# esteinig/sketchy

Measured on AMD Instinct MI355X. Metric: reads/sec streamed (s=10000,k=16,40k-genome ref), higher is better.
Workload: dtype u64

## Files before the change

sketchy_amd/csrc/skx_capi.hip:

```cpp
#include <dlfcn.h>
#include <hip/hip_runtime.h>
#include <rccl/rccl.h>

#include <unistd.h>

#include <algorithm>
#include <atomic>
#include <chrono>
#include <cmath>
#include <condition_variable>
#include <cstdarg>
#include <cstdio>
#include <cstdlib>
#include <cstring>
#include <mutex>
#include <string>
#include <thread>
#include <unordered_map>
#include <vector>

#include "sketchy_hip.h"
#include "skx_common.hpp"
#include "skx_kernels.hpp"

// ... 899 lines not shown
    bool back_pending[2] = {false, false};
    hipEvent_t ev_pslot[3] = {nullptr, nullptr, nullptr};
    bool pslot_pending[3] = {false, false, false};
    int pslot = 0;
    hipEvent_t ev_pairq[2] = {nullptr, nullptr};
    bool pairq_pending[2] = {false, false};
    bool packed = false;
    u32 top_k = 0, max_reads = 0, sk_stride = 0;
    u64 max_bases = 0;
    u32 pcap = 0;
    u32 qcap = 0;
    u64* d_qd = nullptr;
    u32 *d_qrow = nullptr, *d_sslot = nullptr, *d_qinfo = nullptr, *d_qloc = nullptr, *d_cls_bsum = nullptr;
    u32* d_nd_hs = nullptr;
    u32* h_lcount = nullptr;
    u32 lcount_seq = 0, lcount_seen = 0, lcount_floor = 0;
    u32* h_nq_sink = nullptr;
    u32* h_nd = nullptr;
    u32 *d_rowcnt = nullptr;
    u32 *d_gain = nullptr;
    u32 *d_gain_s = nullptr;
    u32 *d_candslot = nullptr;
    u32 *d_candmask = nullptr;
    uint2 *d_lrow = nullptr;
    u32 *d_nlrow = nullptr, *d_gain_l = nullptr, *d_cbase = nullptr, *d_cwl = nullptr, *d_ncwl = nullptr;
    u64 *d_cw = nullptr;
    u64 *d_inb = nullptr, *d_hit = nullptr;
    skx::LongRows long_rows() const { return skx::LongRows{d_lrow, d_nlrow, qcap + 128, d_inb, ref->n_lw}; }
    bool use_pat = false;
    u32 *d_hist = nullptr, *d_nprow = nullptr;
    u64* d_pcw = nullptr;
    u32 npat_pad = 0;
    skx::PatRows pat_rows() const { return skx::PatRows{d_hist, npat_pad, d_gain_l, d_nprow}; }
    skx::RareIndex rare_index() const {
        skx::RareIndex ri = ref->rare_index();
        if (!use_pat) { ri.prec = nullptr; ri.n_pat = 0; }
        if (!static_dense) { ri.qs = nullptr; ri.n_sd = 0; }
        return ri;
    }
    u32 *d_cbad = nullptr, *d_nqc = nullptr;
    u32 *d_spc_g0 = nullptr, *d_spc_grp = nullptr;
    u32 n_pad_c = 0, n_grp_c = 0, cand_seq = 0;
    struct PassSet {
        u64 *tab = nullptr;
        u32 *cand = nullptr;
        u64 *tabc = nullptr;
        u32 *ncand = nullptr;
        u32 *mode = nullptr, *any_full = nullptr, *nqc_total = nullptr;
        u64 *mc = nullptr;
        u64 *mqc = nullptr;
        u64 *rowany_c = nullptr;
        u32 *grp_any_c = nullptr;
        u32 *smap = nullptr;
        u32 *pair_qc = nullptr;
        u32 *nd = nullptr;
        u32 *h_pub = nullptr;
    } ps[2];
    struct PassChains {
        bool pending = false, ranked = false, has_cand = false, update_table = false, forced_full = false, legacy = false;
        SubPass subs[kGroupMax];
        int n_sub = 0, b = 0, slot = 0;
        u32 P = 0, nq_rows = 0, seq = 0;
        u64 nq_est = 0;
    } pcq[2];
    int pc_head = 0, pc_n = 0;
    bool hint_all_overflow = false;
    u32 hint_seq = 0;
    u32 passes_since_fresh = 0;
    bool fresh_table = true;
    u32 legacy_run = 0;
    u64 batches_compact = 0, batches_full = 0;
    bool have_split_hint = false;
    double nd_frac = 1.0;
    u32 qcap_max = 0;
    bool qcap_auto = false;
    u64 qrows_grown = 0;
    u32 coalesce = 1;
    u32 rpass = 0;
    u64 reads_total = 0;
    uint8_t* d_bases = nullptr;
    u64* d_offsets = nullptr;
    u64* d_sk = nullptr;
    u32 *d_len = nullptr, *d_cnt = nullptr, *d_poff = nullptr;
    bool side_ready[kSides] = {};
    u64* sd_sk[kSides] = {};
    u64 pool_cap[kSides] = {};
    u32 pool_fixed = 0;
    u64* sd_rows[kSides] = {};
    u32 cur_stride = 0;
    u32 cur_pool_cap = 0, cur_pool_fixed = 0;
// ... 112 lines not shown
    std::vector<hipEvent_t> ev_pool;
    double ms[SKX_N_STAGES] = {0, 0, 0, 0, 0};
    u64 launches[SKX_N_STAGES] = {0, 0, 0, 0, 0};
};

static void free_side(skx_stream* st, int i);
static void free_lane(skx_stream* st, int i);
static void stream_free(skx_stream* st) {
    if (!st) return;
    (void)hipSetDevice(st->device);
    if (st->hs0) (void)hipStreamSynchronize(st->hs0);
    if (st->hs1) (void)hipStreamSynchronize(st->hs1);
    if (st->hs) (void)hipStreamSynchronize(st->hs);
    if (st->hs2) (void)hipStreamSynchronize(st->hs2);
    for (int i = 1; i < skx_stream::kRankLanes; ++i)
        if (st->lane[i].s) (void)hipStreamSynchronize(st->lane[i].s);
    for (int i = 0; i < kSides; ++i) (void)hipFree(st->sd_rows[i]);
    void* ptrs[] = {st->d_bases, st->d_offsets, st->d_pair_h[0], st->d_pair_h[1],
                    st->d_q[0], st->d_q[1], st->d_pair_r[0], st->d_pair_r[1], st->d_pair_q[0], st->d_pair_q[1],
                    st->d_poff_pass[0], st->d_poff_pass[1], st->d_poff_pass[2], st->d_pair_r[2], st->d_nq[0], st->d_nq[1], st->d_win[0], st->d_win[1], st->d_m, st->d_mint, st->d_mq[0], st->d_mq[1],
                    st->d_topk_idx, st->d_topk_sum, st->d_cons, st->d_ev.n_events, st->d_ev.ev_read, st->d_ev.ev_idx, st->d_ev.ev_sum, st->d_ev.ev_codes, st->d_tab_tmp, st->d_rank_idx, st->d_rank_sum, st->d_bsum, st->d_grp_any[0],
                    st->d_grp_any[1], st->d_hbuf, st->d_wb[0], st->d_wb[1], st->d_rowany[0], st->d_rowany[1], st->d_mqext,
                    st->d_qd, st->d_qrow, st->d_sslot, st->d_qinfo, st->d_qloc, st->d_cls_bsum, st->d_nd_hs,
                    st->d_rowcnt, st->d_gain, st->d_gain_s, st->d_candslot, st->d_candmask, st->d_lrow, st->d_nlrow, st->d_gain_l, st->d_cbase, st->d_cwl, st->d_ncwl, st->d_cw, st->d_cbad, st->d_nqc, st->d_spc_g0, st->d_spc_grp, st->d_inb, st->d_hit, st->d_hist, st->d_nprow, st->d_pcw, st->d_ms[0], st->d_ms[1], st->d_mdirty_s};
    for (auto& q : st->ps) {
        for (void* x : {(void*)q.tab, (void*)q.cand, (void*)q.tabc, (void*)q.ncand, (void*)q.mode, (void*)q.any_full, (void*)q.nqc_total, (void*)q.mc, (void*)q.mqc,
                        (void*)q.rowany_c, (void*)q.grp_any_c, (void*)q.smap, (void*)q.pair_qc, (void*)q.nd}) (void)hipFree(x);
        if (q.h_pub) (void)hipHostFree(q.h_pub);
    }
    for (auto& t : st->d_tab) (void)hipFree(t);
    for (int i = 0; i < skx_stream::kRankLanes; ++i) free_lane(st, i);
    for (int i = 1; i < skx_stream::kRankLanes; ++i)
        if (st->own_lane_stream && st->lane[i].s) (void)hipStreamDestroy(st->lane[i].s);
    for (void* p : ptrs) (void)hipFree(p);
    if (st->h_poff) (void)hipHostFree(st->h_poff);
    if (st->h_offsets) (void)hipHostFree(st->h_offsets);
    if (st->h_nq) (void)hipHostFree(st->h_nq);
    if (st->h_nd) (void)hipHostFree(st->h_nd);
    if (st->h_nq_sink) (void)hipHostFree(st->h_nq_sink);
    if (st->h_lcount) (void)hipHostFree(st->h_lcount);
    if (st->h_chk_base) (void)hipHostFree(st->h_chk_base);
    for (int i = 0; i < kSides; ++i) {
        free_side(st, i);
        if (st->ev_main[i]) (void)hipEventDestroy(st->ev_main[i]);
    }
    if (!st->shared_queues && st->hs1 && st->hs1 != st->hs0) (void)hipStreamDestroy(st->hs1);
    (void)hipFree(st->d_ht[0]); (void)hipFree(st->d_ht[1]); (void)hipFree(st->d_dict_ctr[0]); (void)hipFree(st->d_dict_ctr[1]);
// ... 392 lines not shown
    memset(st->h_nd, 0, 4 * 4);
    SCHK(hipHostMalloc((void**)&st->h_nq_sink, 4 * 4, hipHostMallocCoherent));
    SCHK(hipHostMalloc((void**)&st->h_lcount, 4 * 4, hipHostMallocCoherent));
    memset(st->h_lcount, 0, 4 * 4);
    SCHK(hipMalloc(&st->d_nd_hs, 64));
    SCHK(hipMemset(st->d_nd_hs, 0, 64));
    if (ref->d_kt_key) {
        SCHK(hipMalloc(&st->d_qd, (size_t)st->pcap * 8));
        SCHK(hipMalloc(&st->d_qrow, (size_t)st->pcap * 4));
        SCHK(hipMalloc(&st->d_sslot, (size_t)st->pcap * 8));
        SCHK(hipMalloc(&st->d_qinfo, (size_t)st->pcap * 4));
        SCHK(hipMalloc(&st->d_qloc, (size_t)st->pcap * 4));
        SCHK(hipMalloc(&st->d_cls_bsum, ((size_t)st->pcap / 1024 + 2) * 4));
    }
    {
        const u32 nb = skx::kPassBatchesMax, cap = skx::kCandCap, rows_c = skx::kCandRows;
        st->n_pad_c = n_sp * cap;
        st->n_grp_c = st->n_pad_c / (skx::kRankWords * 64);
        SCHK(hipMalloc(&st->d_rowcnt, (size_t)nb * ((size_t)st->qcap + 128) * 4));
        SCHK(hipMalloc(&st->d_gain, (size_t)nb * n_pad * 4));
        if (ref->d_kt_key) SCHK(hipMalloc(&st->d_gain_s, (size_t)nb * n_pad * 4 * skx::gain_sparse_stride()));
        SCHK(hipMalloc(&st->d_candslot, (size_t)nb * n_pad * 4));
        SCHK(hipMalloc(&st->d_candmask, (size_t)n_pad * 4));
        if (ref->d_mlong) {
            SCHK(hipMalloc(&st->d_lrow, (size_t)nb * ((size_t)st->qcap + 128) * 8));
            SCHK(hipMalloc(&st->d_nlrow, skx::pass_counter_bytes()));
            SCHK(hipMalloc(&st->d_gain_l, (size_t)nb * n_pad * 4));
            SCHK(hipMalloc(&st->d_cw, (size_t)nb * (n_pad / 64) * 8));
            SCHK(hipMalloc(&st->d_cbase, (size_t)nb * (n_pad / 64) * 4));
            SCHK(hipMalloc(&st->d_cwl, (size_t)nb * st->n_pad_c * 4));
            SCHK(hipMalloc(&st->d_ncwl, 64));
            if (ref->d_mlongT) {
                SCHK(hipMalloc(&st->d_inb, (size_t)nb * ref->n_lw * 8));
                SCHK(hipMalloc(&st->d_hit, (size_t)nb * ref->n_lw * 8));
            }
            if (ref->d_prec && ref->n_pat && st->n_grp_c * skx::kRankWords <= skx::pat_words_max()) {
                st->use_pat = true;
                st->npat_pad = (ref->n_pat + 63u) & ~63u;
                SCHK(hipMalloc(&st->d_hist, (size_t)nb * st->npat_pad * 4));
                SCHK(hipMalloc(&st->d_nprow, skx::pass_counter_bytes()));
                SCHK(hipMalloc(&st->d_pcw, (size_t)nb * ref->n_pat * st->n_grp_c * skx::kRankWords * 8));
            }
        }
        SCHK(hipMalloc(&st->d_cbad, 64));
        SCHK(hipMalloc(&st->d_nqc, skx::pass_counter_bytes()));
        std::vector<u32> g0c(n_sp), grpc(st->n_grp_c);
// ... 274 lines not shown
        st->hint_pairs[b] = P;
    }
    if (P == 0) HIPCHK(hipMemsetAsync(d_nd, 0, 16, hs));
    HIPCHK(hipGetLastError());
    if (!inserted) {
        HIPCHK(hipEventRecord(st->ev_skread[st->side], hs));
        st->sk_reader_pending[st->side] = true;
    }
    HIPCHK(hipEventRecord(st->ev_dict[b], hs));

    if (!sdm && ((!st->have_hint && !nq_known && P > 0) || (split_dict && !st->have_split_hint && P > 0))) {
        HIPCHK(hipStreamSynchronize(hs));
        take_hint(b, P);
        st->have_split_hint = true;
        if (!nq_known) nq_est = std::max<u64>(1, hint_nq(b));
    }
    const u64 nd_est = sdm ? std::max<u32>(1u, ref->n_sd) : split_dict ? std::max<u64>(1, (u64)((double)nq_est * st->nd_frac * 1.1) + 64) : nq_est;

    const u32 n_grp_all = n_pad / (skx::kRankWords * 64);
    u32* d_mdirty = d_grp_any + n_grp_all;
    SKX_MARK("pass: dictionary queued", 0);
    HIPCHK(hipMemsetAsync(d_mdirty, 0, 4, hs));
    SKX_MARK("pass: memset mdirty", 0);
    auto wait_back = [&]() -> int {
        if (st->back_pending[b]) { HIPCHK(hipStreamWaitEvent(hs, st->ev_back[b], 0)); st->back_pending[b] = false; }
        HIPCHK(hipMemcpyAsync(ps.nd, d_nd, 16, hipMemcpyDeviceToDevice, hs));
        HIPCHK(hipMemsetAsync(d_grp_any, 0, (size_t)n_grp_all * 4, hs));
        if (P > 0) {
            skx::launch_pair_q(hs, st->d_pair_h[b], P, d_q, d_nq, d_pair_q, split_dict ? st->d_qrow : nullptr, st->d_bbase, st->d_btot, ref->max_ref);
            HIPCHK(hipGetLastError());
        }
        HIPCHK(hipEventRecord(st->ev_pairq[b], hs));
        st->pairq_pending[b] = true;
        return SKX_OK;
    };
    bool ranked = false, all_forced = false, all_ranked = true;
    for (int i = 0; i < n_sub; ++i) {
        const bool r = st->top_k && subs[i].d_topk_idx && subs[i].d_topk_sum;
        ranked = ranked || r; all_ranked = all_ranked && r && !subs[i].d_shared && !subs[i].d_counts;
    }
    const u32* only_if = nullptr;
    u32 seq = 0;
    static const int legacy_env = skx::knob("SKX_TABLE_LEGACY") ? atoi(skx::knob("SKX_TABLE_LEGACY")) : 1 << 30;
    static const int cand_env0 = skx::knob("SKX_CAND") ? atoi(skx::knob("SKX_CAND")) : 1;
    const bool fresh_overflow = st->fresh_table && ref->max_species > skx::kCandCap && st->top_k <= 1;
    const bool second_blind = st->passes_since_fresh == 1 && !((int)(st->lcount_seen - st->lcount_floor) > 0);
    const bool legacy = update_table && all_ranked && cand_env0 && legacy_env > 0 &&
                        (fresh_overflow || (st->hint_all_overflow && !second_blind && (int)st->legacy_run < legacy_env));
    st->legacy_run = legacy ? st->legacy_run + 1 : 0;
    if (update_table) { st->passes_since_fresh = st->fresh_table ? 1 : st->passes_since_fresh + 1; st->fresh_table = false; }
    const bool long_rows = split_dict && ref->d_mlong != nullptr;
    static const int tail_env = skx::knob("SKX_TAIL_SCALE") ? atoi(skx::knob("SKX_TAIL_SCALE")) : 8;
    const u32 walk_scale = st->tail_pass ? (u32)std::max(1, tail_env) : 1u;
    skx::PassBatches pbt;
    pbt.n = (u32)n_sub;
    for (int i = 0; i < n_sub; ++i) pbt.p_off[i] = subs[i].p_off;
    pbt.p_off[n_sub] = P;
    auto rare_gains = [&](hipStream_t on) -> int {
        const skx::RareIndex ri = st->rare_index();
        const skx::LongRows lrows = st->long_rows();
        const skx::PatRows prows = st->pat_rows();
        skx::launch_gain_sparse(on, d_nd, q_bound, st->d_rowcnt, qstride, (u32)n_sub, n_pad, st->d_gain_s, st->d_sslot, ri, long_rows ? &lrows : nullptr, walk_scale,
                                (long_rows && st->use_pat) ? &prows : nullptr);
        if (long_rows) skx::launch_gain_long(on, lrows, ri, d_nd, st->d_rowcnt, qstride, (u32)n_sub, n_pad, st->d_gain_l, walk_scale);
        if (long_rows && st->use_pat)
            skx::launch_gain_dense(on, ri.pm, nullptr, n_pad, ri.d_npat, ri.n_pat, st->d_hist, st->npat_pad, (u32)n_sub, st->d_gain_l);
        HIPCHK(hipGetLastError());
        return SKX_OK;
    };
    auto row_counts = [&]() -> int {
        HIPCHK(hipMemset2DAsync(st->d_rowcnt, (size_t)qstride * 4, 0, (size_t)nq_rows * 4, (size_t)n_sub, hs));
        skx::launch_pass_hist(hs, d_pair_q, pbt, st->d_rowcnt, qstride);
// ... 62 lines not shown
        const u64* m_int = split ? st->d_mint : nullptr;
        HIPCHK(hipMemsetAsync(st->d_gain, 0, (size_t)n_sub * n_pad * 4, hs));
        if (P > 0) {
            SKXCHK(row_counts());
            skx::launch_gain_dense(hs, d_m, m_int, n_pad, d_nd, sdm ? ref->n_sd : q_bound, st->d_rowcnt, qstride, (u32)n_sub, st->d_gain,
                                   (sdm && ref->n_species > 1) ? ref->d_segw : nullptr, ref->d_grp_sp);
            if (split_dict) SKXCHK(rare_gains(hs));
        }
        skx::launch_pass_tables(hs, st->d_cum, st->d_gain, (split_dict && P > 0) ? st->d_gain_s : nullptr,
                                (long_rows && P > 0) ? st->d_gain_l : nullptr, (u32)n_sub, n_pad, ps.tab);
        st->d_cum = ps.tab + (size_t)n_sub * n_pad;
        static const int cand_env = skx::knob("SKX_CAND") ? atoi(skx::knob("SKX_CAND")) : 1;
        static const int hint_env = skx::knob("SKX_CAND_HINT") ? atoi(skx::knob("SKX_CAND_HINT")) : 1;
        (void)hint_env;
        all_forced = !cand_env;
        u32 force_full = all_forced ? 0xFFu : 0u;
        for (int i = 0; i < n_sub; ++i) if (subs[i].d_shared || subs[i].d_counts) force_full |= 1u << i;
        HIPCHK(hipMemsetAsync(st->d_cbad, 0, 64, hs));
        HIPCHK(hipMemsetAsync(st->d_nqc, 0, skx::pass_counter_bytes(), hs));
        const bool pat_rows = st->use_pat && long_rows && ranked && P > 0 && !all_forced;
        if (pat_rows) skx::launch_pat_nqc_init(hs, st->d_nqc, st->npat_pad);
        if (ranked) {
            HIPCHK(hipMemsetAsync(st->d_candmask, 0, (size_t)n_pad * 4, hs));
            skx::launch_cand_select(hs, ps.tab, n_pad, spc, (u32)n_sub, st->top_k, cap, ps.cand, st->d_candslot, ps.tabc, ps.ncand, st->d_cbad,
                                    st->d_candmask);
            HIPCHK(hipMemsetAsync(ps.grp_any_c, 0, (size_t)n_sub * st->n_grp_c * 4, hs));
            if (split_dict && P > 0 && !all_forced) {
                HIPCHK(hipMemsetAsync(ps.mqc, 0, (size_t)n_sub * st->n_grp_c * rows_c * skx::kRankWords * 8, hs));
                HIPCHK(hipMemsetAsync(ps.rowany_c, 0, (size_t)n_sub * st->n_grp_c * (rows_c / 64) * 8, hs));
                HIPCHK(hipMemset2DAsync(ps.smap, (size_t)qstride * 4, 0, (size_t)nq_rows * 4, (size_t)n_sub, hs));
                skx::launch_cand_sparse(hs, st->d_sslot, d_nd, q_bound, st->rare_index(), st->d_candmask, st->d_candslot, n_pad, st->d_cbad, (u32)n_sub, st->d_nqc,
                                        ps.smap, qstride, ps.mqc, (size_t)st->n_grp_c * rows_c * skx::kRankWords, rows_c, ps.rowany_c,
                                        st->n_grp_c * (rows_c / 64), ps.grp_any_c, st->n_grp_c, walk_scale);
                if (long_rows) {
                    const u32 n_gw = n_pad / 64;
                    HIPCHK(hipMemsetAsync(st->d_cw, 0, (size_t)n_sub * n_gw * 8, hs));
                    HIPCHK(hipMemsetAsync(st->d_cbase, 0xFF, (size_t)n_sub * n_gw * 4, hs));
                    HIPCHK(hipMemsetAsync(st->d_ncwl, 0, 64, hs));
                    skx::launch_cand_words(hs, ps.cand, st->n_pad_c, (u32)n_sub, n_gw, st->d_cw, st->d_cbase, st->d_cwl, st->d_ncwl);
                    if (st->d_hit) skx::launch_cand_hit(hs, ps.cand, st->n_pad_c, (u32)n_sub, st->d_cbad, st->rare_index(), st->d_inb, st->d_hit);
                    skx::launch_cand_long(hs, st->long_rows(), st->rare_index(), d_nd, st->d_cw, st->d_cbase, st->d_cwl, st->d_ncwl, st->n_pad_c,
                                          st->d_cbad, (u32)n_sub, st->d_nqc, ps.smap, qstride, ps.mqc, (size_t)st->n_grp_c * rows_c * skx::kRankWords,
                                          rows_c, ps.rowany_c, st->n_grp_c * (rows_c / 64), ps.grp_any_c, st->n_grp_c, walk_scale, st->d_hit);
                }
                if (pat_rows) {
                    const skx::RareIndex ri = st->rare_index();
                    skx::launch_cand_pat_rows(hs, ri, d_nd, st->d_candmask, st->d_candslot, n_pad, st->d_cbad, (u32)n_sub, st->d_pcw, ps.mqc,
                                              (size_t)st->n_grp_c * rows_c * skx::kRankWords, rows_c, ps.rowany_c, st->n_grp_c * (rows_c / 64), ps.grp_any_c,
// ... 1309 lines not shown
    for (u32 g = 0; g < n; ++g)
        if (cur[g] > SKX_MAX_TABLE_SUM || add[g] > SKX_MAX_TABLE_SUM - cur[g])
            return fail(SKX_ERR_INVALID, "skx_stream_table_add: genome %u would hold more than 2^54 - 1 = 18014398509481983", g);
    HIPCHK(hipMemcpyAsync(st->d_tab_tmp, add, (size_t)n * 8, hipMemcpyHostToDevice, st->hs2));
    skx::launch_add_table(st->hs2, st->d_cum, st->d_tab_tmp, n, st->ref->d_real2pad);
    st->fresh_table = false;
    HIPCHK(hipGetLastError());
    HIPCHK(hipStreamSynchronize(st->hs2));
    return SKX_OK;
}
SKX_API int skx_stream_reset(skx_stream* st) {
    if (!st) return fail(SKX_ERR_INVALID, "NULL stream");
    SKXCHK(use_device(st->device));
    SKXCHK(flush_pending(st));
    HIPCHK(hipStreamSynchronize(st->hs0));
    HIPCHK(hipStreamSynchronize(st->hs1));
    HIPCHK(hipStreamSynchronize(st->hs));
    HIPCHK(hipMemsetAsync(st->d_cum, 0, (size_t)st->ref->n_pad * 8, st->hs2));
    HIPCHK(hipStreamSynchronize(st->hs2));
    st->reads_total = 0;
    st->h_nq[2] = 1; st->h_nq[3] = 1;
    st->hint_all_overflow = false;
    st->hint_seq = st->cand_seq;
    st->legacy_run = 0;
    st->lcount_floor = st->lcount_seq;
    st->fresh_table = true;
    st->cum_writer = nullptr;
    return SKX_OK;
}
SKX_API int skx_stream_reads(const skx_stream* st, uint64_t* n_reads) {
    if (!st || !n_reads) return fail(SKX_ERR_INVALID, "NULL argument");
    *n_reads = st->reads_total;
    for (int i = 0; i < st->n_pend; ++i) *n_reads += st->pend[i].n_reads;
    return SKX_OK;
}
SKX_API int skx_stream_stats(skx_stream* st, uint64_t* out, uint32_t n_out) {
    if (!st || !out) return fail(SKX_ERR_INVALID, "NULL argument");
    uint64_t live = 0;
    SKXCHK(use_device(st->device));
    SKXCHK(skx_stream_sync(st));
    {
        const u32 n_grp = st->ref->n_pad / (skx::kRankWords * 64);
        std::vector<u32> flags(n_grp, 0);
        HIPCHK(hipMemcpy(flags.data(), st->d_grp_any[st->buf ^ 1], (size_t)n_grp * 4, hipMemcpyDeviceToHost));
        for (u32 f : flags) live += f ? 1 : 0;
    }
// ... 700 lines not shown
```

sketchy_amd/csrc/skx_kernels.hip:

```cpp
#include <algorithm>
#include <cstdlib>
#include <mutex>
#include <type_traits>

#include "skx_common.hpp"
#include "skx_kernels.hpp"

#ifndef SKX_FEW_CANDS
#define SKX_FEW_CANDS 8
#endif
#ifndef SKX_SCAN_ROWS
#define SKX_SCAN_ROWS 8
#endif
#ifndef SKX_SCAN_OCC
#define SKX_SCAN_OCC 1
#endif
#ifndef SKX_SCAN_SPLIT_READS
#define SKX_SCAN_SPLIT_READS 1
#endif
#ifndef SKX_WALK_BLOCKS
#define SKX_WALK_BLOCKS 256
#endif
#ifndef SKX_GAIN_SPARSE_STRIDE
#define SKX_GAIN_SPARSE_STRIDE 16
#endif
#ifndef SKX_SEGSUM_PRIO
#define SKX_SEGSUM_PRIO 2
// ... 4059 lines not shown
    return theta;
}
__global__ __launch_bounds__(1024) void cand_count_kernel(const u64* __restrict__ t0, const u64* __restrict__ t1, Species sp, u32 top_k,
                                                          u32* __restrict__ d_max, volatile u32* __restrict__ h_out, u32 seq) {
    __builtin_amdgcn_s_setprio(3);
    __shared__ u64 sh64[16];
    __shared__ u32 sh32[16];
    u32 worst = 0;
    for (u32 spi = 0; spi < sp.n_sp; ++spi) {
        const u32 g0 = sp.g0[spi], n = sp.n[spi];
        const u64 theta = species_theta(t0, g0, n, top_k, sh64, sh32);
        u32 c = 0;
        for (u32 g = g0 + threadIdx.x; g < g0 + n; g += 1024u) c += t1[g] >= theta ? 1u : 0u;
        worst = max(worst, block1024_sum_u32(c, sh32));
    }
    if (threadIdx.x == 0u) {
        (void)d_max;
        h_out[0] = worst;
        __threadfence_system();
        h_out[1] = seq;
        __threadfence_system();
    }
}
__global__ __launch_bounds__(1024) void cand_select_kernel(const u64* __restrict__ tab, u32 n_pad, Species sp, u32 top_k, u32 cap,
                                                           u32* __restrict__ cand, u32* __restrict__ candslot, u64* __restrict__ tabc,
                                                           u32* __restrict__ ncand, u32* __restrict__ bad, u32* __restrict__ candmask) {
    __builtin_amdgcn_s_setprio(3);
    __shared__ u64 sh64[16];
    __shared__ u32 sh32[16];
    __shared__ u32 wbase[17];
    const u32 b = blockIdx.x / sp.n_sp, spi = blockIdx.x % sp.n_sp, tid = threadIdx.x, lane = lane_id(), wv = tid >> 6;
    const u32 g0 = sp.g0[spi], n = sp.n[spi];
    const u32 g_end = spi + 1u < sp.n_sp ? sp.g0[spi + 1u] : n_pad;
    const u64* t0 = tab + (size_t)b * n_pad;
    const u64* t1 = t0 + n_pad;
    const u64 theta = species_theta(t0, g0, n, top_k, sh64, sh32);
    u32 base = 0;
    u32* my_cand = cand + (size_t)(b * sp.n_sp + spi) * cap;
    u64* my_tabc = tabc + (size_t)b * sp.n_sp * cap + (size_t)spi * cap;
    for (u32 c0 = g0; c0 < g_end; c0 += 1024u) {
        const u32 g = c0 + tid;
        const bool is = g < g0 + n && t1[g] >= theta;
        const u64 bal = __ballot(is);
        const u32 before = (u32)__popcll(bal & lanemask_lt()), wtot = (u32)__popcll(bal);
        __syncthreads();
        if (lane == 0u) wbase[wv] = wtot;
        __syncthreads();
        u32 wb = 0, tot = 0;
#pragma unroll
        for (u32 i = 0; i < 16u; ++i) { const u32 v = wbase[i]; wb += i < wv ? v : 0u; tot += v; }
        const u32 pos = base + wb + before;
        if (g < g_end) {
            u32 slot = kCandNone;
            if (is && pos < cap) { my_cand[pos] = g; my_tabc[pos] = t0[g]; slot = spi * cap + pos; atomicOr(&candmask[g], 1u << b); }
            candslot[(size_t)b * n_pad + g] = slot;
        }
        base += tot;
    }
    for (u32 i = min(base, cap) + tid; i < cap; i += 1024u) { my_cand[i] = kCandNone; my_tabc[i] = 0; }
    if (tid == 0u) {
        ncand[b * sp.n_sp + spi] = min(base, cap);
        if (base > cap) atomicOr(&bad[b], 1u);
    }
}
__global__ __launch_bounds__(256) void cand_gather_m_kernel(const u64* __restrict__ m_bits, const u64* __restrict__ m_int, u32 n_pad,
// ... 548 lines not shown
                      u32* gain_l, u32 walk_scale) {
    hipLaunchKernelGGL(gain_long_kernel, dim3(cdiv(ri.n_gw, 64), n_b, (u32)env_int("SKX_G_GAINLONG", 8) * std::min(4u, std::max(1u, walk_scale))), dim3(256), 0, st, lr, ri, n_d, cnt, row_stride, n_pad, gain_l);
}
void launch_mlong_transpose(hipStream_t st, const u64* mlong, u32 n_long, u32 n_gw, u64* mlongT, u32 n_lw) {
    if (n_long == 0) return;
    hipLaunchKernelGGL(mlong_transpose_kernel, dim3(n_lw, cdiv(n_gw, 4)), dim3(256), 0, st, mlong, n_long, n_gw, mlongT, n_lw);
}
void launch_cand_hit(hipStream_t st, const u32* cand, u32 n_pad_c, u32 n_b, const u32* bad, const RareIndex& ri, const u64* inb, u64* hit) {
    hipLaunchKernelGGL(cand_hit_kernel, dim3(cdiv(n_pad_c, 4), n_b), dim3(256), 0, st, cand, n_pad_c, bad, ri, inb, hit);
}
void launch_cand_words(hipStream_t st, const u32* cand, u32 n_pad_c, u32 n_b, u32 n_gw, u64* cw, u32* cbase, u32* cwl, u32* ncwl) {
    hipLaunchKernelGGL(cand_words_kernel, dim3(n_b), dim3(1024), 0, st, cand, n_pad_c, n_gw, cw, cbase, cwl, ncwl);
}
void launch_cand_long(hipStream_t st, const LongRows& lr, const RareIndex& ri, const u32* n_d, const u64* cw, const u32* cbase, const u32* cwl,
                      const u32* ncwl, u32 n_pad_c, u32* bad, u32 n_b, u32* nqc, u32* smap, u32 smap_stride, u64* mqc, size_t mqc_stride,
                      u32 rows_c, u64* rowany_c, u32 rowany_stride, u32* grp_any_c, u32 n_grp_c, u32 walk_scale, const u64* hit) {
    hipLaunchKernelGGL(cand_long_kernel, dim3((u32)env_int("SKX_G_CANDLONG", 192) * std::min(4u, std::max(1u, walk_scale)), n_b), dim3(256), 0, st, lr, ri, n_d, cw, cbase, cwl, ncwl, n_pad_c, bad, nqc, smap, smap_stride, mqc,
                       mqc_stride, rows_c, rowany_c, rowany_stride, grp_any_c, n_grp_c, hit);
}
void launch_pass_tables(hipStream_t st, const u64* prev, const u32* gain, const u32* gain_s, const u32* gain_l, u32 n_b, u32 n_pad, u64* tab) {
    hipLaunchKernelGGL(pass_tables_kernel, dim3(cdiv(n_pad, 256)), dim3(256), 0, st, prev, gain, gain_s, gain_l, n_b, n_pad, tab);
}
void launch_cand_select(hipStream_t st, const u64* tab, u32 n_pad, const Species& sp, u32 n_b, u32 top_k, u32 cap, u32* cand, u32* candslot,
                        u64* tabc, u32* ncand, u32* bad, u32* candmask) {
    hipLaunchKernelGGL(cand_select_kernel, dim3(n_b * sp.n_sp), dim3(1024), 0, st, tab, n_pad, sp, top_k, cap, cand, candslot, tabc, ncand, bad, candmask);
}
void launch_cand_count(hipStream_t st, const u64* t0, const u64* t1, const Species& sp, u32 top_k, u32* h_out, u32 seq) {
    hipLaunchKernelGGL(cand_count_kernel, dim3(1), dim3(1024), 0, st, t0, t1, sp, top_k, nullptr, h_out, seq);
}
void launch_cand_gather_m(hipStream_t st, const u64* m_bits, const u64* m_int, u32 n_pad, const u32* n_d, u32 rows_bound, const u32* cand, u32 n_pad_c,
                          const u32* bad, u32 n_b, u64* mc, u32 words_c) {
    const u32 words = std::min(words_c, std::max(1u, cdiv(rows_bound, 64)));
    hipLaunchKernelGGL(cand_gather_m_kernel, dim3(cdiv(n_pad_c, 256), words, n_b), dim3(256), 0, st, m_bits, m_int, n_pad, n_d, cand, n_pad_c, bad, mc, words_c);
}
void launch_cand_sparse(hipStream_t st, const u32* sslot, const u32* n_d, u32 rows_bound, const RareIndex& ri, const u32* candmask,
                        const u32* candslot, u32 n_pad, u32* bad, u32 n_b, u32* nqc, u32* smap, u32 smap_stride, u64* mqc, size_t mqc_stride,
                        u32 rows_c, u64* rowany_c, u32 rowany_stride, u32* grp_any_c, u32 n_grp_c, u32 walk_scale) {
    hipLaunchKernelGGL(cand_sparse_kernel, dim3(std::max(1u, std::min(cdiv(rows_bound, 256), kWalkBlocks * std::max(1u, walk_scale)))), dim3(256), 0, st, sslot, n_d, ri, candmask,
                       candslot, n_pad, bad, n_b, nqc, smap, smap_stride, mqc, mqc_stride, rows_c, rowany_c, rowany_stride, grp_any_c, n_grp_c);
}
void launch_cand_publish(hipStream_t st, const u32* bad, u32 force_full, const u32* ncand, const u32* nqc, const u32* n_d, u32 n_b, u32 n_sp,
                         u32 rows_c, u32* mode, u32* any_full, u32* nqc_total, u32* h_pub, u32 seq) {
    hipLaunchKernelGGL(cand_publish_kernel, dim3(1), dim3(1), 0, st, bad, force_full, ncand, nqc, n_d, n_b, n_sp, rows_c, mode, any_full, nqc_total,
                       h_pub, seq);
}
void launch_m_clear(hipStream_t st, u64* m_bits, u64* m_int, u32 n_pad, const u32* n_d, const u32* any_full) {
    hipLaunchKernelGGL(m_clear_kernel, dim3(512), dim3(256), 0, st, m_bits, m_int, n_pad, n_d, any_full);
}
// ... 653 lines not shown
```

sketchy_amd/csrc/skx_kernels.hpp:

```cpp
#pragma once
#include <hip/hip_runtime.h>
#include <stddef.h>
#include <stdint.h>

#include <stdlib.h>

namespace skx {
typedef unsigned long long u64;
typedef unsigned int u32;

inline const char* knob(const char* name) {
#ifdef SKX_EXPERIMENTS
    return getenv(name);
#else
    (void)name;
    return nullptr;
#endif
}

constexpr int kSketchCap = 2048;
constexpr u32 kSegLen = 64;
constexpr int kRankWords = 8;

struct Species { const u32* g0; const u32* n; const u32* of_grp; u32 n_sp; };
// ... 69 lines not shown
void launch_sparse_fill(hipStream_t st, const u32* sslot, const u32* n_d, const RareIndex& ri, u64* m_bits, u32 n_pad, u32* m_dirty,
                        u32 rows_bound, const u32* only_if = nullptr );
void launch_nd_from_nq(hipStream_t st, const u32* n_q, u32* n_d, u32* h_words);

static const u32 kPassBatchesMax = 8;
static const u32 kCandCap = 1024;
static const u32 kCandRows = 131072;
struct PassBatches { u32 n; u32 p_off[kPassBatchesMax + 1]; };
void launch_pass_hist(hipStream_t st, const u32* pair_q, const PassBatches& pb, u32* cnt, u32 row_stride);
void launch_gain_dense(hipStream_t st, const u64* m_bits, const u64* m_int , u32 n_pad, const u32* n_d, u32 rows_bound, const u32* cnt,
                       u32 row_stride, u32 n_b, u32* gain, const u32* segw = nullptr ,
                       const u32* grp_sp = nullptr);
void launch_gain_sparse(hipStream_t st, const u32* n_d, u32 rows_bound, const u32* cnt, u32 row_stride, u32 n_b, u32 n_pad, u32* gain_s,
                        const u32* sslot, const RareIndex& ri, const LongRows* lr, u32 walk_scale, const PatRows* pr = nullptr);
void launch_pat_nqc_init(hipStream_t st, u32* nqc, u32 v);
void launch_cand_pat_rows(hipStream_t st, const RareIndex& ri, const u32* n_d, const u32* candmask, const u32* candslot, u32 n_pad, u32* bad, u32 n_b,
                          u64* pcw, u64* mqc, size_t mqc_stride, u32 rows_c, u64* rowany_c, u32 rowany_stride, u32* grp_any_c, u32 n_grp_c);
void launch_cand_pat_map(hipStream_t st, const LongRows& lr, const PatRows& pr, const RareIndex& ri, const u32* n_d, const u32* candmask,
                         const u32* candslot, u32 n_pad, u32* bad, u32 n_b, u32* nqc, u32* smap, u32 smap_stride, const u64* pcw, u64* mqc,
                         size_t mqc_stride, u32 rows_c, u64* rowany_c, u32 rowany_stride, u32* grp_any_c, u32 n_grp_c, u32 rows_bound, u32 walk_scale = 1);
u32 gain_sparse_stride();
void launch_pass_tables(hipStream_t st, const u64* prev, const u32* gain, const u32* gain_s , const u32* gain_l , u32 n_b,
                        u32 n_pad, u64* tab);
void launch_cand_select(hipStream_t st, const u64* tab, u32 n_pad, const Species& sp, u32 n_b, u32 top_k, u32 cap, u32* cand, u32* candslot,
                        u64* tabc, u32* ncand, u32* bad, u32* candmask);
void launch_cand_count(hipStream_t st, const u64* t0, const u64* t1, const Species& sp, u32 top_k, u32* h_out, u32 seq);
void launch_cand_gather_m(hipStream_t st, const u64* m_bits, const u64* m_int , u32 n_pad, const u32* n_d, u32 rows_bound, const u32* cand,
                          u32 n_pad_c, const u32* bad, u32 n_b, u64* mc, u32 words_c);
void launch_cand_sparse(hipStream_t st, const u32* sslot, const u32* n_d, u32 rows_bound, const RareIndex& ri, const u32* candmask,
                        const u32* candslot, u32 n_pad, u32* bad, u32 n_b, u32* nqc, u32* smap, u32 smap_stride, u64* mqc, size_t mqc_stride,
                        u32 rows_c, u64* rowany_c, u32 rowany_stride, u32* grp_any_c, u32 n_grp_c, u32 walk_scale = 1);
void launch_cand_publish(hipStream_t st, const u32* bad, u32 force_full, const u32* ncand, const u32* nqc, const u32* n_d, u32 n_b, u32 n_sp,
                         u32 rows_c, u32* mode, u32* any_full, u32* nqc_total, u32* h_pub, u32 seq);
void launch_m_clear(hipStream_t st, u64* m_bits, u64* m_int , u32 n_pad, const u32* n_d, const u32* any_full);
void launch_cand_pair_rows(hipStream_t st, const u32* pair_q, u32 n_pairs, const u32* n_d, const u32* smap, u32 rows_c, u32* pair_qc);
void launch_cand_rows_back(hipStream_t st, u32* out_idx, u32 n_reads, u32 n_sp, u32 top_k, const u32* cand, u32 cap, const u32* g0);
constexpr u32 kConsensusTopMax = 64;
void launch_consensus_rows(hipStream_t st, const u32* idx, u64 first_row, u64 n_rows, u32 n_sp, u32 top_k, const u32* g0, const u32* codes,
                           u32 n_feat, u32* out, u32 n_code_rows);
constexpr u32 kChangeWidthMax = 4096;
void launch_change_flags(hipStream_t st, const u32* rows, u32 width, u32 ra, u32 rb, u32* flag);
void launch_change_events(hipStream_t st, const u32* flag, u32* pos, u32* bsum, u32 n, u32 cap, u32* n_events, u32* ev_read,
                          const u32* idx, const u64* sum, u32 w_idx, u32* ev_idx, u64* ev_sum, const u32* codes, u32 w_codes, u32* ev_codes);

void launch_pair_q(hipStream_t st, const u64* pair_h, u32 n_pairs, const u64* q, const u32* n_q, u32* pair_q, const u32* qrow ,
                   const u32* bbase, const u32* btot, u64 max_ref );
static const int kPairBaseMax = 7;
struct PairBase { const u32* p[kPairBaseMax] = {}; };
// ... 99 lines not shown
```

Before: 149.0 million.

## Prune candidate genomes with a pivot-genome bound before candidate selection

For top-1 streams with species larger than the candidate cap, a new pivot rule picks the current best genome per large species and counts per-read hits for it against the sketch matrix. It then keeps only genomes whose score bounds could still overtake the pivot, so fewer genomes overflow into the candidate set. For single-species references it also skips the forced legacy full-table path on fresh tables. The aim is to avoid falling back to the expensive full/legacy pass, at the cost of three extra kernels and per-read binary searches into the matrix.

```diff
diff --git a/sketchy_amd/csrc/skx_cand_rule.hpp b/sketchy_amd/csrc/skx_cand_rule.hpp
--- /dev/null
+++ b/sketchy_amd/csrc/skx_cand_rule.hpp
@@ -0,0 +1,25 @@
+#pragma once
+#include <stdint.h>
+
+#if defined(__HIPCC__)
+#define SKX_RULE_HD __host__ __device__
+#else
+#define SKX_RULE_HD
+#endif
+
+namespace skx {
+
+template <class CcAt, class PAt>
+SKX_RULE_HD inline bool cand_pivot_keep(uint64_t s_g, uint64_t e_g, uint32_t n_reads, CcAt cc, PAt p) {
+    const uint64_t d = e_g - s_g;
+    uint32_t lo = 0, hi = n_reads;
+    while (lo < hi) {
+        const uint32_t mid = lo + (hi - lo + 1u) / 2u;
+        if ((uint64_t)cc(mid) <= d) lo = mid; else hi = mid - 1u;
+    }
+    const uint32_t i = lo;
+    if (i >= 1u && s_g + (uint64_t)cc(i) >= (uint64_t)p(i)) return true;
+    return i < n_reads && e_g >= (uint64_t)p(i + 1u);
+}
+
+}
diff --git a/sketchy_amd/csrc/skx_capi.hip b/sketchy_amd/csrc/skx_capi.hip
--- a/sketchy_amd/csrc/skx_capi.hip
+++ b/sketchy_amd/csrc/skx_capi.hip
@@ -945,6 +945,9 @@
     u32 *d_gain_s = nullptr;
     u32 *d_candslot = nullptr;
     u32 *d_candmask = nullptr;
+    u32 *d_pv_species = nullptr, *d_pv_pivot = nullptr, *d_pv_hits = nullptr, *d_pv_bsum = nullptr;
+    u64* d_pv_keep = nullptr;
+    u32 n_pvbig = 0, pv_max_n = 0;
     uint2 *d_lrow = nullptr;
     u32 *d_nlrow = nullptr, *d_gain_l = nullptr, *d_cbase = nullptr, *d_cwl = nullptr, *d_ncwl = nullptr;
     u64 *d_cw = nullptr;
@@ -989,6 +992,7 @@
     int pc_head = 0, pc_n = 0;
     bool hint_all_overflow = false;
     u32 hint_seq = 0;
+    u32 hint_floor = 0;
     u32 passes_since_fresh = 0;
     bool fresh_table = true;
     u32 legacy_run = 0;
@@ -1147,7 +1151,7 @@
                     st->d_topk_idx, st->d_topk_sum, st->d_cons, st->d_ev.n_events, st->d_ev.ev_read, st->d_ev.ev_idx, st->d_ev.ev_sum, st->d_ev.ev_codes, st->d_tab_tmp, st->d_rank_idx, st->d_rank_sum, st->d_bsum, st->d_grp_any[0],
                     st->d_grp_any[1], st->d_hbuf, st->d_wb[0], st->d_wb[1], st->d_rowany[0], st->d_rowany[1], st->d_mqext,
                     st->d_qd, st->d_qrow, st->d_sslot, st->d_qinfo, st->d_qloc, st->d_cls_bsum, st->d_nd_hs,
-                    st->d_rowcnt, st->d_gain, st->d_gain_s, st->d_candslot, st->d_candmask, st->d_lrow, st->d_nlrow, st->d_gain_l, st->d_cbase, st->d_cwl, st->d_ncwl, st->d_cw, st->d_cbad, st->d_nqc, st->d_spc_g0, st->d_spc_grp, st->d_inb, st->d_hit, st->d_hist, st->d_nprow, st->d_pcw, st->d_ms[0], st->d_ms[1], st->d_mdirty_s};
+                    st->d_rowcnt, st->d_gain, st->d_gain_s, st->d_candslot, st->d_candmask, st->d_pv_species, st->d_pv_pivot, st->d_pv_hits, st->d_pv_bsum, st->d_pv_keep, st->d_lrow, st->d_nlrow, st->d_gain_l, st->d_cbase, st->d_cwl, st->d_ncwl, st->d_cw, st->d_cbad, st->d_nqc, st->d_spc_g0, st->d_spc_grp, st->d_inb, st->d_hit, st->d_hist, st->d_nprow, st->d_pcw, st->d_ms[0], st->d_ms[1], st->d_mdirty_s};
     for (auto& q : st->ps) {
         for (void* x : {(void*)q.tab, (void*)q.cand, (void*)q.tabc, (void*)q.ncand, (void*)q.mode, (void*)q.any_full, (void*)q.nqc_total, (void*)q.mc, (void*)q.mqc,
                         (void*)q.rowany_c, (void*)q.grp_any_c, (void*)q.smap, (void*)q.pair_qc, (void*)q.nd}) (void)hipFree(x);
@@ -1586,6 +1590,21 @@
         if (ref->d_kt_key) SCHK(hipMalloc(&st->d_gain_s, (size_t)nb * n_pad * 4 * skx::gain_sparse_stride()));
         SCHK(hipMalloc(&st->d_candslot, (size_t)nb * n_pad * 4));
         SCHK(hipMalloc(&st->d_candmask, (size_t)n_pad * 4));
+        if (st->top_k == 1 && (u64)st->rpass + 1 <= (u64)skx::kPivotBlocksMax * skx::kPivotBlockReads) {
+            std::vector<u32> big;
+            for (u32 sp = 0; sp < n_sp && big.size() < skx::kPivotSpecies; ++sp)
+                if (ref->sp_n[sp] > cap) big.push_back(sp);
+            if (!big.empty()) {
+                st->n_pvbig = (u32)big.size();
+                SCHK(hipMalloc(&st->d_pv_species, big.size() * 4));
+                SCHK(hipMemcpy(st->d_pv_species, big.data(), big.size() * 4, hipMemcpyHostToDevice));
+                SCHK(hipMalloc(&st->d_pv_pivot, (size_t)nb * big.size() * 4));
+                SCHK(hipMalloc(&st->d_pv_hits, (size_t)nb * big.size() * ((size_t)st->rpass + 2) * 4));
+                SCHK(hipMalloc(&st->d_pv_bsum, (size_t)nb * big.size() * skx::kPivotBlocksMax * 4));
+                SCHK(hipMalloc(&st->d_pv_keep, (size_t)nb * (n_pad / 64) * 8));
+                for (u32 sp : big) st->pv_max_n = std::max(st->pv_max_n, ref->sp_n[sp]);
+            }
+        }
         if (ref->d_mlong) {
             SCHK(hipMalloc(&st->d_lrow, (size_t)nb * ((size_t)st->qcap + 128) * 8));
             SCHK(hipMalloc(&st->d_nlrow, skx::pass_counter_bytes()));
@@ -1906,6 +1925,12 @@
     SKX_MARK("pass: dictionary queued", 0);
     HIPCHK(hipMemsetAsync(d_mdirty, 0, 4, hs));
     SKX_MARK("pass: memset mdirty", 0);
+    bool pivot_rule = false;
+    auto pairs_consumed = [&]() -> int {
+        HIPCHK(hipEventRecord(st->ev_pairq[b], hs));
+        st->pairq_pending[b] = true;
+        return SKX_OK;
+    };
     auto wait_back = [&]() -> int {
         if (st->back_pending[b]) { HIPCHK(hipStreamWaitEvent(hs, st->ev_back[b], 0)); st->back_pending[b] = false; }
         HIPCHK(hipMemcpyAsync(ps.nd, d_nd, 16, hipMemcpyDeviceToDevice, hs));
@@ -1914,8 +1939,7 @@
             skx::launch_pair_q(hs, st->d_pair_h[b], P, d_q, d_nq, d_pair_q, split_dict ? st->d_qrow : nullptr, st->d_bbase, st->d_btot, ref->max_ref);
             HIPCHK(hipGetLastError());
         }
-        HIPCHK(hipEventRecord(st->ev_pairq[b], hs));
-        st->pairq_pending[b] = true;
+        if (!pivot_rule) SKXCHK(pairs_consumed());
         return SKX_OK;
     };
     bool ranked = false, all_forced = false, all_ranked = true;
@@ -1927,11 +1951,18 @@
     u32 seq = 0;
     static const int legacy_env = skx::knob("SKX_TABLE_LEGACY") ? atoi(skx::knob("SKX_TABLE_LEGACY")) : 1 << 30;
     static const int cand_env0 = skx::knob("SKX_CAND") ? atoi(skx::knob("SKX_CAND")) : 1;
-    const bool fresh_overflow = st->fresh_table && ref->max_species > skx::kCandCap && st->top_k <= 1;
-    const bool second_blind = st->passes_since_fresh == 1 && !((int)(st->lcount_seen - st->lcount_floor) > 0);
+    static const bool pivot_env = !skx::knob("SKX_CAND_PIVOT") || atoi(skx::knob("SKX_CAND_PIVOT")) != 0;
+    static const bool fresh_legacy_env = skx::knob("SKX_FRESH_LEGACY") && atoi(skx::knob("SKX_FRESH_LEGACY")) != 0;
+    const bool pivot_stream = pivot_env && st->n_pvbig > 0 && st->top_k == 1 && cand_env0;
+    const bool select_first = pivot_stream && ref->n_species == 1 && !fresh_legacy_env;
+    const bool fresh_overflow = st->fresh_table && ref->max_species > skx::kCandCap && st->top_k <= 1 && !select_first;
+    const bool first_published = select_first && (int)(st->hint_seq - st->hint_floor) > 0;
+    const bool second_blind = st->passes_since_fresh == 1 && !((int)(st->lcount_seen - st->lcount_floor) > 0) && !first_published;
     const bool legacy = update_table && all_ranked && cand_env0 && legacy_env > 0 &&
                         (fresh_overflow || (st->hint_all_overflow && !second_blind && (int)st->legacy_run < legacy_env));
     st->legacy_run = legacy ? st->legacy_run + 1 : 0;
+    pivot_rule = pivot_stream && update_table && !legacy && ranked && P > 0;
+    for (int i = 0; i < n_sub; ++i) pivot_rule = pivot_rule && subs[i].rb - subs[i].ra <= st->rpass;
     if (update_table) { st->passes_since_fresh = st->fresh_table ? 1 : st->passes_since_fresh + 1; st->fresh_table = false; }
     const bool long_rows = split_dict && ref->d_mlong != nullptr;
     static const int tail_env = skx::knob("SKX_TAIL_SCALE") ? atoi(skx::knob("SKX_TAIL_SCALE")) : 8;
@@ -2040,8 +2071,20 @@
         if (pat_rows) skx::launch_pat_nqc_init(hs, st->d_nqc, st->npat_pad);
         if (ranked) {
             HIPCHK(hipMemsetAsync(st->d_candmask, 0, (size_t)n_pad * 4, hs));
+            skx::PivotRule piv{};
+            if (pivot_rule) {
+                piv.species = st->d_pv_species; piv.n_big = st->n_pvbig; piv.pivot = st->d_pv_pivot; piv.hits = st->d_pv_hits; piv.bsum = st->d_pv_bsum; piv.keep = st->d_pv_keep;
+                piv.r_stride = st->rpass + 2;
+                for (int i = 0; i < n_sub; ++i) {
+                    piv.poff[i] = subs[i].d_poff; piv.p_off[i] = subs[i].p_off; piv.p_base[i] = subs[i].p_base; piv.n_reads[i] = subs[i].rb - subs[i].ra;
+                }
+                skx::launch_pivot(hs, ps.tab, n_pad, spc, (u32)n_sub, cap, piv);
+                skx::launch_pivot_hits(hs, st->d_pair_h[b], ref->d_mat, ref->s, ref->d_exc_g, ref->d_exc_h, ref->n_exc, (u32)n_sub, piv);
+                SKXCHK(pairs_consumed());
+                skx::launch_pivot_keep(hs, ps.tab, n_pad, spc, (u32)n_sub, st->pv_max_n, piv);
+            }
             skx::launch_cand_select(hs, ps.tab, n_pad, spc, (u32)n_sub, st->top_k, cap, ps.cand, st->d_candslot, ps.tabc, ps.ncand, st->d_cbad,
-                                    st->d_candmask);
+                                    st->d_candmask, pivot_rule ? &piv : nullptr);
             HIPCHK(hipMemsetAsync(ps.grp_any_c, 0, (size_t)n_sub * st->n_grp_c * 4, hs));
             if (split_dict && P > 0 && !all_forced) {
                 HIPCHK(hipMemsetAsync(ps.mqc, 0, (size_t)n_sub * st->n_grp_c * rows_c * skx::kRankWords * 8, hs));
@@ -3397,6 +3440,7 @@
     st->h_nq[2] = 1; st->h_nq[3] = 1;
     st->hint_all_overflow = false;
     st->hint_seq = st->cand_seq;
+    st->hint_floor = st->cand_seq;
     st->legacy_run = 0;
     st->lcount_floor = st->lcount_seq;
     st->fresh_table = true;
diff --git a/sketchy_amd/csrc/skx_kernels.hip b/sketchy_amd/csrc/skx_kernels.hip
--- a/sketchy_amd/csrc/skx_kernels.hip
+++ b/sketchy_amd/csrc/skx_kernels.hip
@@ -3,6 +3,7 @@
 #include <mutex>
 #include <type_traits>
 
+#include "skx_cand_rule.hpp"
 #include "skx_common.hpp"
 #include "skx_kernels.hpp"
 
@@ -4108,9 +4109,135 @@
         __threadfence_system();
     }
 }
+__global__ __launch_bounds__(1024) void pivot_kernel(const u64* __restrict__ tab, u32 n_pad, Species sp, u32 cap, PivotRule piv) {
+    __builtin_amdgcn_s_setprio(3);
+    __shared__ u64 sh64[16];
+    __shared__ u32 sh32[16];
+    const u32 b = blockIdx.x / piv.n_big, j = blockIdx.x % piv.n_big, spi = piv.species[j];
+    const u32 g0 = sp.g0[spi], n = sp.n[spi];
+    const u64* t0 = tab + (size_t)b * n_pad;
+    const u64* t1 = tab + (size_t)(b + 1u) * n_pad;
+    {
+        const u64 theta = species_theta(t0, g0, n, 1u, sh64, sh32);
+        u32 c = 0;
+        for (u32 g = g0 + threadIdx.x; g < g0 + n; g += 1024u) c += t1[g] >= theta ? 1u : 0u;
+        if (block1024_sum_u32(c, sh32) <= cap || theta == 0) {
+            if (threadIdx.x == 0u) piv.pivot[b * piv.n_big + j] = kCandNone;
+            return;
+        }
+    }
+    u64 m = 0;
+    for (u32 g = g0 + threadIdx.x; g < g0 + n; g += 1024u) m = max(m, t1[g]);
+    m = block1024_max_u64(m, sh64);
+    u64 best = 0;
+    for (u32 g = g0 + threadIdx.x; g < g0 + n; g += 1024u)
+        if (t1[g] == m) { best = (u64)(0xFFFFFFFFu - g); break; }
+    best = block1024_max_u64(best, sh64);
+    if (threadIdx.x == 0u) piv.pivot[b * piv.n_big + j] = n ? 0xFFFFFFFFu - (u32)best : kCandNone;
+}
+__device__ __forceinline__ bool genome_holds(const u64* __restrict__ mat, u32 s, u32 g, u64 h, const u32* __restrict__ exc_g,
+                                             const u64* __restrict__ exc_h, u32 n_exc) {
+    if (h >= kEmpty) {
+        for (u32 e = 0; e < n_exc; ++e)
+            if (exc_h[e] == h && exc_g[e] == g) return true;
+        return false;
+    }
+    const u64* col = mat + (size_t)(g / kTileGenomes) * s * kTileGenomes + g % kTileGenomes;
+    u32 lo = 0, hi = s;
+    while (lo < hi) {
+        const u32 mid = (lo + hi) >> 1;
+        if (col[(size_t)mid * kTileGenomes] < h) lo = mid + 1u; else hi = mid;
+    }
+    return lo < s && col[(size_t)lo * kTileGenomes] == h;
+}
+__global__ __launch_bounds__(256) void pivot_hits_kernel(const u64* __restrict__ pair_h, const u64* __restrict__ mat, u32 s,
+                                                         const u32* __restrict__ exc_g, const u64* __restrict__ exc_h, u32 n_exc,
+                                                         PivotRule piv) {
+    static_assert(kPivotBlockReads == 256u, "one read per thread");
+    __builtin_amdgcn_s_setprio(3);
+    __shared__ u32 wtot[kPivotSpecies][4];
+    const u32 b = blockIdx.y, nr = piv.n_reads[b], r = blockIdx.x * 256u + threadIdx.x;
+    if (blockIdx.x * 256u > nr) return;
+    u32 c[kPivotSpecies];
+#pragma unroll
+    for (u32 j = 0; j < kPivotSpecies; ++j) c[j] = 0;
+    if (r < nr) {
+        const u32* poff = piv.poff[b];
+        const u64* ph = pair_h + piv.p_off[b];
+        for (u32 p = poff[r] - piv.p_base[b], pe = poff[r + 1u] - piv.p_base[b]; p < pe; ++p) {
+            const u64 h = ph[p];
+#pragma unroll
+            for (u32 j = 0; j < kPivotSpecies; ++j) {
+                if (j < piv.n_big) {
+                    const u32 g = piv.pivot[b * piv.n_big + j];
+                    if (g != kCandNone && genome_holds(mat, s, g, h, exc_g, exc_h, n_exc)) c[j] += 1u;
+                }
+            }
+        }
+    }
+    const u32 lane = lane_id(), wv = threadIdx.x >> 6;
+    u32 incl[kPivotSpecies];
+#pragma unroll
+    for (u32 j = 0; j < kPivotSpecies; ++j) {
+        incl[j] = wave_incl_scan(c[j]);
+        if (lane == 63u) wtot[j][wv] = incl[j];
+    }
+    __syncthreads();
+#pragma unroll
+    for (u32 j = 0; j < kPivotSpecies; ++j) {
+        if (j < piv.n_big) {
+            u32 before = 0, total = 0;
+#pragma unroll
+            for (u32 w = 0; w < 4u; ++w) { before += w < wv ? wtot[j][w] : 0u; total += wtot[j][w]; }
+            const size_t bj = (size_t)b * piv.n_big + j;
+            if (r <= nr) piv.hits[bj * piv.r_stride + r] = before + incl[j] - c[j];
+            if (threadIdx.x == 0u) piv.bsum[bj * kPivotBlocksMax + blockIdx.x] = total;
+        }
+    }
+}
+__global__ __launch_bounds__(256) void pivot_keep_kernel(const u64* __restrict__ tab, u32 n_pad, Species sp, PivotRule piv) {
+    __builtin_amdgcn_s_setprio(3);
+    __shared__ u32 bpre[kPivotBlocksMax];
+    __shared__ u32 wtot[4];
+    const u32 b = blockIdx.y / piv.n_big, j = blockIdx.y % piv.n_big, spi = piv.species[j], tid = threadIdx.x;
+    const u32 g0 = sp.g0[spi], n = sp.n[spi];
+    const size_t bj = (size_t)b * piv.n_big + j;
+    const u32 pg = piv.pivot[bj];
+    if (pg == kCandNone || blockIdx.x * 256u >= n) return;
+    const u32 nr = piv.n_reads[b], n_blk = nr / kPivotBlockReads + 1u;
+    static_assert(kPivotBlocksMax == 4096u, "sixteen block totals per thread");
+    {
+        const u32* bs = piv.bsum + bj * kPivotBlocksMax;
+        u32 mine = 0;
+        for (u32 i = 0; i < 16u; ++i) mine += tid * 16u + i < n_blk ? bs[tid * 16u + i] : 0u;
+        const u32 incl = wave_incl_scan(mine), wv = tid >> 6;
+        if (lane_id() == 63u) wtot[wv] = incl;
+        __syncthreads();
+        u32 run = incl - mine;
+        for (u32 w = 0; w < 4u; ++w) run += w < wv ? wtot[w] : 0u;
+        for (u32 i = 0; i < 16u; ++i) {
+            if (tid * 16u + i < n_blk) { bpre[tid * 16u + i] = run; run += bs[tid * 16u + i]; }
+        }
+        __syncthreads();
+    }
+    const u64* t0 = tab + (size_t)b * n_pad;
+    const u64* t1 = t0 + n_pad;
+    const u32* poff = piv.poff[b];
+    const u32 p_base = piv.p_base[b];
+    const u32* hits = piv.hits + bj * piv.r_stride;
+    const u64 s_p = t0[pg];
+    auto cc_at = [&](u32 i) -> u64 { return (u64)(poff[i] - p_base); };
+    auto p_at = [&](u32 i) -> u64 { return s_p + hits[i] + bpre[i / kPivotBlockReads]; };
+    const bool rule = p_at(nr) == t1[pg];
+    const u32 g = g0 + blockIdx.x * 256u + tid;
+    const bool keep = g < g0 + n && (!rule || cand_pivot_keep(t0[g], t1[g], nr, cc_at, p_at));
+    const u64 bal = __ballot(keep);
+    if (lane_id() == 0u) piv.keep[(size_t)b * (n_pad / 64u) + g / 64u] = bal;
+}
 __global__ __launch_bounds__(1024) void cand_select_kernel(const u64* __restrict__ tab, u32 n_pad, Species sp, u32 top_k, u32 cap,
                                                            u32* __restrict__ cand, u32* __restrict__ candslot, u64* __restrict__ tabc,
-                                                           u32* __restrict__ ncand, u32* __restrict__ bad, u32* __restrict__ candmask) {
+                                                           u32* __restrict__ ncand, u32* __restrict__ bad, u32* __restrict__ candmask,
+                                                           PivotRule piv) {
     __builtin_amdgcn_s_setprio(3);
     __shared__ u64 sh64[16];
     __shared__ u32 sh32[16];
@@ -4121,12 +4248,15 @@
     const u64* t0 = tab + (size_t)b * n_pad;
     const u64* t1 = t0 + n_pad;
     const u64 theta = species_theta(t0, g0, n, top_k, sh64, sh32);
+    const u64* keep = nullptr;
+    for (u32 j = 0; j < piv.n_big; ++j)
+        if (piv.species[j] == spi && piv.pivot[b * piv.n_big + j] != kCandNone) keep = piv.keep + (size_t)b * (n_pad / 64u);
     u32 base = 0;
     u32* my_cand = cand + (size_t)(b * sp.n_sp + spi) * cap;
     u64* my_tabc = tabc + (size_t)b * sp.n_sp * cap + (size_t)spi * cap;
     for (u32 c0 = g0; c0 < g_end; c0 += 1024u) {
         const u32 g = c0 + tid;
-        const bool is = g < g0 + n && t1[g] >= theta;
+        const bool is = g < g0 + n && t1[g] >= theta && (!keep || ((keep[g >> 6] >> (g & 63u)) & 1ull));
         const u64 bal = __ballot(is);
         const u32 before = (u32)__popcll(bal & lanemask_lt()), wtot = (u32)__popcll(bal);
         __syncthreads();
@@ -4721,8 +4851,25 @@
     hipLaunchKernelGGL(pass_tables_kernel, dim3(cdiv(n_pad, 256)), dim3(256), 0, st, prev, gain, gain_s, gain_l, n_b, n_pad, tab);
 }
 void launch_cand_select(hipStream_t st, const u64* tab, u32 n_pad, const Species& sp, u32 n_b, u32 top_k, u32 cap, u32* cand, u32* candslot,
-                        u64* tabc, u32* ncand, u32* bad, u32* candmask) {
-    hipLaunchKernelGGL(cand_select_kernel, dim3(n_b * sp.n_sp), dim3(1024), 0, st, tab, n_pad, sp, top_k, cap, cand, candslot, tabc, ncand, bad, candmask);
+                        u64* tabc, u32* ncand, u32* bad, u32* candmask, const PivotRule* piv) {
+    PivotRule none{};
+    hipLaunchKernelGGL(cand_select_kernel, dim3(n_b * sp.n_sp), dim3(1024), 0, st, tab, n_pad, sp, top_k, cap, cand, candslot, tabc, ncand, bad, candmask,
+                       (piv && top_k <= 1u) ? *piv : none);
+}
+void launch_pivot(hipStream_t st, const u64* tab, u32 n_pad, const Species& sp, u32 n_b, u32 cap, const PivotRule& piv) {
+    if (piv.n_big == 0 || n_b == 0) return;
+    hipLaunchKernelGGL(pivot_kernel, dim3(n_b * piv.n_big), dim3(1024), 0, st, tab, n_pad, sp, cap, piv);
+}
+void launch_pivot_keep(hipStream_t st, const u64* tab, u32 n_pad, const Species& sp, u32 n_b, u32 max_genomes, const PivotRule& piv) {
+    if (piv.n_big == 0 || n_b == 0 || max_genomes == 0) return;
+    hipLaunchKernelGGL(pivot_keep_kernel, dim3(cdiv(max_genomes, 256), n_b * piv.n_big), dim3(256), 0, st, tab, n_pad, sp, piv);
+}
+void launch_pivot_hits(hipStream_t st, const u64* pair_h, const u64* mat, u32 s, const u32* exc_g, const u64* exc_h, u32 n_exc, u32 n_b,
+                       const PivotRule& piv) {
+    if (piv.n_big == 0 || n_b == 0) return;
+    u32 nr_max = 0;
+    for (u32 b = 0; b < n_b; ++b) nr_max = std::max(nr_max, piv.n_reads[b]);
+    hipLaunchKernelGGL(pivot_hits_kernel, dim3(nr_max / kPivotBlockReads + 1u, n_b), dim3(256), 0, st, pair_h, mat, s, exc_g, exc_h, n_exc, piv);
 }
 void launch_cand_count(hipStream_t st, const u64* t0, const u64* t1, const Species& sp, u32 top_k, u32* h_out, u32 seq) {
     hipLaunchKernelGGL(cand_count_kernel, dim3(1), dim3(1024), 0, st, t0, t1, sp, top_k, nullptr, h_out, seq);
diff --git a/sketchy_amd/csrc/skx_kernels.hpp b/sketchy_amd/csrc/skx_kernels.hpp
--- a/sketchy_amd/csrc/skx_kernels.hpp
+++ b/sketchy_amd/csrc/skx_kernels.hpp
@@ -115,8 +115,27 @@
 u32 gain_sparse_stride();
 void launch_pass_tables(hipStream_t st, const u64* prev, const u32* gain, const u32* gain_s , const u32* gain_l , u32 n_b,
                         u32 n_pad, u64* tab);
+struct PivotRule;
 void launch_cand_select(hipStream_t st, const u64* tab, u32 n_pad, const Species& sp, u32 n_b, u32 top_k, u32 cap, u32* cand, u32* candslot,
-                        u64* tabc, u32* ncand, u32* bad, u32* candmask);
+                        u64* tabc, u32* ncand, u32* bad, u32* candmask, const PivotRule* piv = nullptr);
+static const u32 kPivotSpecies = 4;
+static const u32 kPivotBlockReads = 256;
+static const u32 kPivotBlocksMax = 4096;
+struct PivotRule {
+    const u32* species;
+    u32 n_big;
+    u32* pivot;
+    u32* hits;
+    u32* bsum;
+    u32 r_stride;
+    u64* keep;
+    const u32* poff[kPassBatchesMax];
+    u32 p_off[kPassBatchesMax], p_base[kPassBatchesMax], n_reads[kPassBatchesMax];
+};
+void launch_pivot(hipStream_t st, const u64* tab, u32 n_pad, const Species& sp, u32 n_b, u32 cap, const PivotRule& piv);
+void launch_pivot_hits(hipStream_t st, const u64* pair_h, const u64* mat, u32 s, const u32* exc_g, const u64* exc_h, u32 n_exc, u32 n_b,
+                       const PivotRule& piv);
+void launch_pivot_keep(hipStream_t st, const u64* tab, u32 n_pad, const Species& sp, u32 n_b, u32 max_genomes, const PivotRule& piv);
 void launch_cand_count(hipStream_t st, const u64* t0, const u64* t1, const Species& sp, u32 top_k, u32* h_out, u32 seq);
 void launch_cand_gather_m(hipStream_t st, const u64* m_bits, const u64* m_int , u32 n_pad, const u32* n_d, u32 rows_bound, const u32* cand,
                           u32 n_pad_c, const u32* bad, u32 n_b, u64* mc, u32 words_c);
```

After: 146.1 million. 1.9% lower.
